# charlesyou999648/ARCO

Hardware: AMD Instinct MI355X
Metric: train steps/sec, ACDC 2D 256x256 bs=16 (higher is better)
Workload: dtype f32; 1 GPU; ACDC 2D 256x256 bs=16 per GPU on 1xMI355X, stratified sampler + 4096-key/class queue (BASELINE.json configs[1]), reference-default flags; classes=4, rep_dim=496, num_queries=256, num_negatives=512, func=smc, apply_aug=cutmix, loss_terms=k1*contrastive + k3*unsupervised + CE + Dice + k2*equivariance (k2 = 1), graph_train=1, parallelism=dp1

## Files before the change

arco_amd/csrc/conv_sp.hip:

```cpp
#include "igemm_args.h"
#include <stdlib.h>
#include <type_traits>

#include "sp_util.h"
__device__ __attribute__((aligned(64))) unsigned int conv_sp_zero_row[32];

template <int A_T, int C_T>
struct SpGeom {
  static constexpr int TH = 4 * A_T, HR = TH + 2, AROWS = HR * 18, BN = C_T * 16;
  static constexpr int A_DW = AROWS * 24;
  static constexpr int NBI = (2 * BN * 6 + 255) / 256;
  static constexpr int SLOT_DW = NBI * 256 * 4;
  static constexpr int NA_IT = (AROWS * 4 + 255) / 256;
  static constexpr int BIAS_DW = 256;
  static constexpr size_t LDS_BYTES = (size_t)(2 * A_DW + 5 * SLOT_DW + BIAS_DW) * 4;
};

template <int A_T, int C_T, bool PRO = false>
__global__ __launch_bounds__(512) void conv3x3_sp_kernel(IgemmArgs a) {
  using G = SpGeom<A_T, C_T>;
  constexpr int TH = G::TH, BN = G::BN, NA = G::NA_IT, NB = G::NBI;
  constexpr int NA4 = (NA + 3) / 4;
  constexpr int NL = NA + (PRO ? 4 : 0);
  extern __shared__ __attribute__((aligned(16))) float smem[];
  unsigned* const As = reinterpret_cast<unsigned*>(smem);
  unsigned* const Bs = As + 2 * G::A_DW;
  float* const bias_s = reinterpret_cast<float*>(Bs + 5 * G::SLOT_DW);

  const int tid = threadIdx.x & 255, lane = tid & 63, wid = tid >> 6, li = lane & 15, g = lane >> 4;
  const bool producer = threadIdx.x >= 256;
  const int tiles_x = a.W >> 4, tiles_y = a.H / TH, tiles_img = tiles_x * tiles_y;
  const int nchunks = a.K >> 4;
  const int total_tiles = a.n_mblocks * a.n_nblocks;
  const bool xcd_map = (gridDim.x & 7) == 0;
  const int G8 = xcd_map ? (int)gridDim.x >> 3 : (int)gridDim.x;
  const int T8 = xcd_map ? (total_tiles + 7) >> 3 : total_tiles;
  const int tile0 = xcd_map ? ((int)blockIdx.x & 7) * T8 + ((int)blockIdx.x >> 3) : (int)blockIdx.x;
  const int tile_end_x = xcd_map ? min(total_tiles, (((int)blockIdx.x & 7) + 1) * T8) : total_tiles;
  const int my_tiles = tile0 < tile_end_x ? (tile_end_x - tile0 + G8 - 1) / G8 : 0;
  const int total_gc = my_tiles * nchunks;
  if (my_tiles == 0) return;
  const bool has_stats = a.stat_sum != nullptr;

  struct Desc { int j, c, img, y0, x0, nblk, mblk, grp; };
  const int ipg = PRO ? a.NB / (a.pro.groups > 1 ? a.pro.groups : 1) : 1;
  auto decode = [&](Desc& d) {
    const int v = tile0 + d.j * G8;
    d.mblk = v / a.n_nblocks; d.nblk = v - d.mblk * a.n_nblocks;
    d.img = d.mblk / tiles_img;
    d.grp = PRO ? d.img / ipg : 0;
    const int r = d.mblk - d.img * tiles_img, ty = r / tiles_x;
    d.y0 = ty * TH; d.x0 = (r - ty * tiles_x) * 16;
  };
  auto advance = [&](Desc& d) { if (++d.c == nchunks) { d.c = 0; ++d.j; decode(d); } };
  Desc d0{0, 0, 0, 0, 0, 0, 0, 0};
  decode(d0);

  if (producer) {
    Desc d1 = d0; advance(d1);
    Desc d2 = d1; advance(d2);
    Desc d3 = d2; advance(d3);
    const int qA = tid & 3;
    int ldsA[NA]; unsigned voff[NA]; int poff[NA];
    unsigned m_valid = 0, m_top = 0, m_bot = 0, m_left = 0, m_right = 0;
#pragma unroll
    for (int it = 0; it < NA; ++it) {
      const int row = (tid + it * 256) >> 2;
      const int hy = row / 18, hx = row - hy * 18;
      const bool valid = row < G::AROWS;
      poff[it] = hy * a.W + hx;
      ldsA[it] = valid ? row * 24 + qA * 2 : -1;
      voff[it] = valid ? (unsigned)(((hy * a.W + hx) * (int)a.lda + qA * 4) * 4) : 0u;
      m_valid |= valid ? (1u << it) : 0u;
      m_top |= (valid && hy == 0) ? (1u << it) : 0u; m_bot |= (valid && hy == TH + 1) ? (1u << it) : 0u;
      m_left |= (valid && hx == 0) ? (1u << it) : 0u; m_right |= (valid && hx == 17) ? (1u << it) : 0u;
    }
    const unsigned safe_off = (unsigned)(((a.W + 1) * (int)a.lda + qA * 4) * 4);
    int woff[NB], wq[NB], wtap[NB];
#pragma unroll
    for (int i = 0; i < NB; ++i) {
      const int p = (i * 4 + wid) * 64 + lane;
      const int tl_ = p / (BN * 6), rem = p - tl_ * (BN * 6), n = rem / 6, q6 = rem - n * 6;
      wtap[i] = tl_ < 2 ? tl_ : 2;
      woff[i] = tl_ < 2 ? ((tl_ * a.Npad + n) * a.Kg) * 24 + q6 * 4 : 0;
      wq[i] = q6 * 4;
    }
    const long wslot2 = (long)2 * a.Npad * a.Kg * 24;
    const float* const zrow = reinterpret_cast<const float*>(conv_sp_zero_row);

    f32x4 ra[2][NA]; unsigned okm2[2] = {0, 0};
    f32x4 rp[2][4]; unsigned ebase2[2] = {0, 0}; bool bord2[2] = {true, true};
    const float* const pm_ = PRO ? uniform_ptr(a.pro.mean) : nullptr; const float* const pi_ = PRO ? uniform_ptr(a.pro.istd) : nullptr;
    const float* const pg_ = PRO ? uniform_ptr(a.pro.gamma) : nullptr; const float* const pb_ = PRO ? uniform_ptr(a.pro.beta) : nullptr;
    const bool pdrop = PRO && a.pro.drop_mode == 1;
    uint32_t dkey = 0, dthr = 0; float keep_scale = 1.f;
    u32x2 salt = {0u, 0u};
    if (PRO && pdrop && a.pro.seed_dev) {
      const float* sp_ = uniform_ptr(reinterpret_cast<const float*>(a.pro.seed_dev));
      asm volatile("global_load_dwordx2 %0, %1, %2" : "=v"(salt) : "v"(0u), "s"(sp_) : "memory");
    }
    auto drop_setup = [&]() {
      if (PRO && pdrop) {
        asm volatile("" : "+v"(salt)::"memory");
        const unsigned long long sv = ((unsigned long long)salt[1] << 32) | salt[0];
        const unsigned long long sd = a.pro.seed_dev ? a.pro.seed ^ (sv * 0x9E3779B97F4A7C15ull) : a.pro.seed;
        dkey = drop_key32(sd); dthr = drop_thr16(a.pro.p); keep_scale = 1.0f / (1.0f - a.pro.p);
      }
    };
    auto load_A = [&](const Desc& d, bool real, int set) {
      const float* gbase = uniform_ptr(real ? a.A + ((((long)d.img * a.H + d.y0 - 1) * a.W + d.x0 - 1) * a.lda + d.c * 16) : a.A);
      unsigned bad = (d.y0 == 0 ? m_top : 0u) | (d.y0 + TH == a.H ? m_bot : 0u) | (d.x0 == 0 ? m_left : 0u) | (d.x0 + 16 == a.W ? m_right : 0u);
      if (!real) bad = ~0u;
      const unsigned okm = m_valid & ~bad;
      okm2[set] = okm;
      const bool border = !real || d.y0 == 0 || d.y0 + TH == a.H || d.x0 == 0 || d.x0 + 16 == a.W;
      if constexpr (PRO) bord2[set] = border;
      if (!border) {
#pragma unroll
        for (int it = 0; it < NA; ++it) asm volatile("global_load_dwordx4 %0, %1, %2" : "=v"(ra[set][it]) : "v"(voff[it]), "s"(gbase) : "memory");
      } else {
#pragma unroll
        for (int it = 0; it < NA; ++it) {
          const unsigned o = ((okm >> it) & 1u) ? voff[it] : safe_off;
          asm volatile("global_load_dwordx4 %0, %1, %2" : "=v"(ra[set][it]) : "v"(o), "s"(gbase) : "memory");
        }
      }
      if constexpr (PRO) {
        const int ch = d.c * 16 + qA * 4;
        const unsigned po = (unsigned)(((real ? d.grp : 0) * a.K + ch) * 4), pa = (unsigned)(ch * 4);
        asm volatile("global_load_dwordx4 %0, %1, %2" : "=v"(rp[set][0]) : "v"(po), "s"(pm_) : "memory");
        asm volatile("global_load_dwordx4 %0, %1, %2" : "=v"(rp[set][1]) : "v"(po), "s"(pi_) : "memory");
        asm volatile("global_load_dwordx4 %0, %1, %2" : "=v"(rp[set][2]) : "v"(pa), "s"(pg_) : "memory");
        asm volatile("global_load_dwordx4 %0, %1, %2" : "=v"(rp[set][3]) : "v"(pa), "s"(pb_) : "memory");
        ebase2[set] = (unsigned)((((d.img * a.H + d.y0 - 1) * a.W + d.x0 - 1) * a.K) + ch);
      }
    };
    auto ra_fence = [&](int set) {
#pragma unroll
      for (int it = 0; it < NA; ++it) asm volatile("" : "+v"(ra[set][it])::"memory");
      if constexpr (PRO) {
#pragma unroll
        for (int j = 0; j < 4; ++j) asm volatile("" : "+v"(rp[set][j])::"memory");
      }
    };
    auto store_A = [&](unsigned* buf, int it, int set) {
      f32x4 v = ra[set][it];
      if constexpr (PRO) {
        v = pro_bn_lrelu(v, ProQuad{rp[set][0], rp[set][1], rp[set][2], rp[set][3]}, a.pro.slope);
        if (pdrop) v = pro_dropout(v, dkey, ebase2[set] + (unsigned)poff[it] * (unsigned)a.K, dthr, keep_scale);
        if (bord2[set]) v = pro_mask(v, okm2[set] >> it);
      } else {
        v = ((okm2[set] >> it) & 1u) ? v : f32x4{0, 0, 0, 0};
      }
      u32x2 p0, p1, p2;
      split3_bf16x4(v, p0, p1, p2);
      if (ldsA[it] >= 0) {
        unsigned* d = buf + ldsA[it];
        *reinterpret_cast<u32x2_ma*>(d) = p0; *reinterpret_cast<u32x2_ma*>(d + 8) = p1; *reinterpret_cast<u32x2_ma*>(d + 16) = p2;
      }
    };
    auto refill = [&](int slot, const Desc& d) {
      const float* base = a.Wp + slot * wslot2 + ((long)d.nblk * BN * a.Kg + d.c) * 24;
#pragma unroll
      for (int i = 0; i < NB; ++i) {
        const bool zero = wtap[i] == 2 || (slot == 4 && wtap[i] == 1);
        const float* src = zero ? zrow + wq[i] : base + woff[i];
        unsigned* dst = Bs + slot * G::SLOT_DW + (i * 4 + wid) * 256;
        __builtin_amdgcn_global_load_lds((glb_void_t*)src, (lds_void_t*)dst, 16, 0, 0);
      }
    };

    for (int i = tid; i < G::BIAS_DW; i += 256) bias_s[i] = (a.bias && i < a.N) ? a.bias[i] : 0.f;
    load_A(d0, true, 0);
    refill(0, d0); refill(1, d0); refill(2, d0);
    wait_vm<3 * NB>();
    drop_setup();
    ra_fence(0);
#pragma unroll
    for (int it = 0; it < NA; ++it) store_A(As, it, 0);
    refill(3, d0);
    load_A(d1, total_gc > 1, 1);
    load_A(d2, total_gc > 2, 0);
    wait_vm<NL>();
    wait_lgkm0();
    __builtin_amdgcn_s_barrier();

    auto pchunk = [&](auto SET_, int gc) {
      constexpr int SET = decltype(SET_)::value;
      const bool more = gc + 1 < total_gc;
      unsigned* Anxt = As + ((gc + 1) & 1) * G::A_DW;
      auto step = [&](auto S_) {
        constexpr int S = decltype(S_)::value;
        constexpr int NS = S <= 2 ? NL + 2 * NB : 2 * NB;
        wait_vm<NS>();
        wait_lgkm0();
        __builtin_amdgcn_s_barrier();
        refill(S == 0 ? 4 : S - 1, S == 0 ? d0 : (more ? d1 : d0));
        if (S == 0) ra_fence(SET);
        if (S <= 3) {
#pragma unroll
          for (int it = S * NA4; it < (S + 1) * NA4 && it < NA; ++it) store_A(Anxt, it, SET);
        }
        if (S == 4) load_A(d3, gc + 3 < total_gc, SET);
      };
      step(std::integral_constant<int, 0>{});
      step(std::integral_constant<int, 1>{});
      step(std::integral_constant<int, 2>{});
      step(std::integral_constant<int, 3>{});
      step(std::integral_constant<int, 4>{});
      d0 = d1; d1 = d2; d2 = d3; advance(d3);
    };
    for (int gc = 0; gc < total_gc; gc += 2) {
      pchunk(std::integral_constant<int, 1>{}, gc);
      if (gc + 1 < total_gc) pchunk(std::integral_constant<int, 0>{}, gc + 1);
    }
    wait_vm<0>();
    return;
  }

  const int tl = g >> 1;
  int aoff[5];
#pragma unroll
  for (int s = 0; s < 5; ++s) {
    const int tap = 2 * s + tl > 8 ? 8 : 2 * s + tl;
    aoff[s] = ((tap / 3) * 18 + tap % 3) * 24;
  }
  const int laneA = (wid * A_T * 18 + li) * 24 + (g & 1) * 4;
  const int laneB = (tl * BN + li) * 24 + (g & 1) * 4;
  bf16x8 fa[2][A_T][3], fb[2][3];
  f32x4 acc[A_T][C_T];
#pragma unroll
  for (int i = 0; i < A_T; ++i)
#pragma unroll
    for (int j = 0; j < C_T; ++j) acc[i][j] = f32x4{0, 0, 0, 0};

  __builtin_amdgcn_s_barrier();
#pragma unroll
  for (int at = 0; at < A_T; ++at)
#pragma unroll
    for (int pl = 0; pl < 3; ++pl) fa[0][at][pl] = lds_bf16x8(As + laneA + aoff[0] + at * 18 * 24 + 8 * pl);
#pragma unroll
  for (int pl = 0; pl < 3; ++pl) fb[0][pl] = lds_bf16x8(Bs + laneB + 8 * pl);

  auto chunk = [&](auto CP_, int gc) {
    constexpr int CP = decltype(CP_)::value;
    const unsigned* Acur = As + (gc & 1) * G::A_DW;
    const unsigned* Anxt = As + ((gc + 1) & 1) * G::A_DW;
    auto step = [&](auto S_) {
      constexpr int S = decltype(S_)::value;
      constexpr int P = (CP + S) & 1, Q = P ^ 1;
      wait_lgkm0();
      __builtin_amdgcn_s_barrier();
      constexpr int NCH = A_T * C_T;
      constexpr int APC = (A_T * 3 + (NCH - 2) - 1) / (NCH - 2 > 0 ? NCH - 2 : 1);
      const unsigned* An = S < 4 ? Acur : Anxt;
#pragma unroll
      for (int ct = 0; ct < C_T; ++ct) {
        constexpr int GB = (C_T & 1) ? (CP + S) : 0;
        const int BPc = (GB + ct) & 1, BPn = BPc ^ 1;
        const bool last = ct + 1 == C_T;
#pragma unroll
        for (int pl = 0; pl < 3; ++pl)
          fb[BPn][pl] = lds_bf16x8(Bs + (last ? (S + 1) % 5 : S) * G::SLOT_DW + laneB + (last ? 0 : ct + 1) * 16 * 24 + 8 * pl);
        __builtin_amdgcn_sched_barrier(0);
#pragma unroll
        for (int at = 0; at < A_T; ++at) {
          mfma_acc(acc[at][ct], fb[BPc][0], fa[P][at][2]);
          mfma_acc(acc[at][ct], fb[BPc][2], fa[P][at][0]);
          mfma_acc(acc[at][ct], fb[BPc][1], fa[P][at][1]);
          mfma_acc(acc[at][ct], fb[BPc][0], fa[P][at][1]);
          mfma_acc(acc[at][ct], fb[BPc][1], fa[P][at][0]);
          mfma_acc(acc[at][ct], fb[BPc][0], fa[P][at][0]);
          const int chain = ct * A_T + at;
#pragma unroll
          for (int k = chain * APC; k < (chain + 1) * APC && k < A_T * 3; ++k)
            fa[Q][k / 3][k % 3] = lds_bf16x8(An + laneA + aoff[(S + 1) % 5] + (k / 3) * 18 * 24 + 8 * (k % 3));
          __builtin_amdgcn_sched_barrier(0);
        }
      }
    };
    step(std::integral_constant<int, 0>{});
    step(std::integral_constant<int, 1>{});
    step(std::integral_constant<int, 2>{});
    step(std::integral_constant<int, 3>{});
    step(std::integral_constant<int, 4>{});
  };

  auto tile_end = [&]() {
    asm volatile("s_nop 15\n\ts_nop 15" ::: "memory");
    const int n0 = d0.nblk * BN;
    float s1[C_T][4], s2[C_T][4];
#pragma unroll
    for (int ct = 0; ct < C_T; ++ct) {
      const int n = n0 + ct * 16 + 4 * g;
      const f32x4 bv = *reinterpret_cast<const f32x4*>(bias_s + n);
#pragma unroll
      for (int r = 0; r < 4; ++r) { s1[ct][r] = 0.f; s2[ct][r] = 0.f; }
#pragma unroll
      for (int at = 0; at < A_T; ++at) {
        const long pix = ((long)d0.img * a.H + d0.y0 + wid * A_T + at) * a.W + d0.x0 + li;
        f32x4 v = acc[at][ct] + bv;
        if (a.R) v += *reinterpret_cast<const f32x4*>(a.R + pix * a.ldr + n);
        *reinterpret_cast<f32x4*>(a.C + pix * a.ldc + n) = v;
#pragma unroll
        for (int r = 0; r < 4; ++r) { s1[ct][r] += v[r]; s2[ct][r] += v[r] * v[r]; }
        acc[at][ct] = f32x4{0, 0, 0, 0};
      }
    }
    if (has_stats) {
      const long slab = (long)d0.mblk * 4 + wid, nslab = (long)a.n_mblocks * 4;
#pragma unroll
      for (int ct = 0; ct < C_T; ++ct)
#pragma unroll
        for (int r = 0; r < 4; ++r) {
          const float v1 = row16_sum(s1[ct][r]), v2 = row16_sum(s2[ct][r]);
          if (li == 0) {
            a.stat_sum[(n0 + ct * 16 + 4 * g + r) * nslab + slab] = v1;
            a.stat_sq[(n0 + ct * 16 + 4 * g + r) * nslab + slab] = v2;
          }
        }
    }
  };

  for (int gc = 0; gc < total_gc; gc += 2) {
    chunk(std::integral_constant<int, 0>{}, gc);
    if (d0.c + 1 == nchunks) tile_end();
    advance(d0);
    if (gc + 1 < total_gc) {
      chunk(std::integral_constant<int, 1>{}, gc + 1);
      if (d0.c + 1 == nchunks) tile_end();
      advance(d0);
    }
  }
}

template <int A_T, int C_T, int NCW = 4>
struct RwGeom {
  static constexpr int TH = NCW * A_T, AROWS = (TH + 2) * 18, BN = C_T * 16;
  static constexpr int A_DW = AROWS * 24;
  static constexpr int WCH_DW = 10 * BN * 24;
  static constexpr int NA_IT = (AROWS * 4 + 255) / 256;
  static constexpr int BIAS_DW = 64;
  static size_t lds_bytes(int nchunks) { return (size_t)(2 * A_DW + nchunks * WCH_DW + BIAS_DW) * 4; }
};

template <int A_T, int C_T, bool PRO = false, int NCW = 4>
__global__ __launch_bounds__((NCW + 4) * 64) void conv3x3_rw_kernel(IgemmArgs a) {
  using G = RwGeom<A_T, C_T, NCW>;
  constexpr int TH = G::TH, BN = G::BN, NA = G::NA_IT;
  constexpr int NL = NA + (PRO ? 4 : 0);
  extern __shared__ __attribute__((aligned(16))) float smem[];
  unsigned* const As = reinterpret_cast<unsigned*>(smem);
  const int nchunks = (a.K + 15) >> 4;
  unsigned* const Ws = As + 2 * G::A_DW;
  float* const bias_s = reinterpret_cast<float*>(Ws + nchunks * G::WCH_DW);
  const bool producer = threadIdx.x >= NCW * 64;
  const int tid = producer ? (int)threadIdx.x - NCW * 64 : (int)threadIdx.x, lane = tid & 63, wid = tid >> 6, li = lane & 15, g = lane >> 4;
  const int tiles_x = a.W >> 4, tiles_y = a.H / TH, tiles_img = tiles_x * tiles_y;
  const int total_tiles = a.n_mblocks;
  const bool xcd_map = (gridDim.x & 7) == 0;
  const int G8 = xcd_map ? (int)gridDim.x >> 3 : (int)gridDim.x;
  const int T8 = xcd_map ? (total_tiles + 7) >> 3 : total_tiles;
  const int tile0 = xcd_map ? ((int)blockIdx.x & 7) * T8 + ((int)blockIdx.x >> 3) : (int)blockIdx.x;
  const int tile_end_x = xcd_map ? min(total_tiles, (((int)blockIdx.x & 7) + 1) * T8) : total_tiles;
  const int my_tiles = tile0 < tile_end_x ? (tile_end_x - tile0 + G8 - 1) / G8 : 0;
  const int total_gc = my_tiles * nchunks;
  if (my_tiles == 0) return;
  const bool has_stats = a.stat_sum != nullptr;
  struct Desc { int j, c, img, y0, x0, mblk, grp; };
  const int ipg = PRO ? a.NB / (a.pro.groups > 1 ? a.pro.groups : 1) : 1;
  auto decode = [&](Desc& d) {
    d.mblk = tile0 + d.j * G8;
    d.img = d.mblk / tiles_img;
    d.grp = PRO ? d.img / ipg : 0;
    const int r = d.mblk - d.img * tiles_img, ty = r / tiles_x;
    d.y0 = ty * TH; d.x0 = (r - ty * tiles_x) * 16;
  };
  auto advance = [&](Desc& d) { if (++d.c == nchunks) { d.c = 0; ++d.j; decode(d); } };
  Desc d0{0, 0, 0, 0, 0, 0, 0};
  decode(d0);

  if (producer) {
    const float* const zrow = reinterpret_cast<const float*>(conv_sp_zero_row);
    const int wpieces = nchunks * 10 * BN * 6;
    for (int p0 = wid * 64; p0 < wpieces; p0 += 256) {
      const int p = p0 + lane;
      const int q6 = p % 6, row = p / 6, n = row % BN, tp = (row / BN) % 10, c = row / (BN * 10);
      const float* src = (tp < 9 && p < wpieces) ? a.Wp + (((long)tp * a.Npad + n) * a.Kg + c) * 24 + q6 * 4 : zrow + q6 * 4;
      __builtin_amdgcn_global_load_lds((glb_void_t*)src, (lds_void_t*)(Ws + p0 * 4), 16, 0, 0);
    }
    for (int i = tid; i < G::BIAS_DW; i += 256) bias_s[i] = (a.bias && i < a.N) ? a.bias[i] : 0.f;
    Desc d1 = d0; advance(d1);
    Desc d2 = d1; advance(d2);
    Desc d3 = d2; advance(d3);
    const int qA = tid & 3;
    int ldsA[NA]; unsigned voff[NA]; int poff[NA];
    unsigned m_valid = 0, m_top = 0, m_bot = 0, m_left = 0, m_right = 0;
#pragma unroll
    for (int it = 0; it < NA; ++it) {
      const int row = (tid + it * 256) >> 2;
      const int hy = row / 18, hx = row - hy * 18;
      const bool valid = row < G::AROWS;
      poff[it] = hy * a.W + hx;
      ldsA[it] = valid ? row * 24 + qA * 2 : -1;
      voff[it] = valid ? (unsigned)(((hy * a.W + hx) * (int)a.lda + qA * 4) * 4) : 0u;
      m_valid |= valid ? (1u << it) : 0u;
      m_top |= (valid && hy == 0) ? (1u << it) : 0u; m_bot |= (valid && hy == TH + 1) ? (1u << it) : 0u;
      m_left |= (valid && hx == 0) ? (1u << it) : 0u; m_right |= (valid && hx == 17) ? (1u << it) : 0u;
    }
    const unsigned safe_off = (unsigned)(((a.W + 1) * (int)a.lda + qA * 4) * 4);
    f32x4 ra[2][NA]; unsigned okm2[2] = {0, 0};
    f32x4 rp[2][4]; unsigned ebase2[2] = {0, 0}; bool bord2[2] = {true, true};
    const float* const pm_ = PRO ? uniform_ptr(a.pro.mean) : nullptr; const float* const pi_ = PRO ? uniform_ptr(a.pro.istd) : nullptr;
    const float* const pg_ = PRO ? uniform_ptr(a.pro.gamma) : nullptr; const float* const pb_ = PRO ? uniform_ptr(a.pro.beta) : nullptr;
    const bool pdrop = PRO && a.pro.drop_mode == 1;
    uint32_t dkey = 0, dthr = 0; float keep_scale = 1.f;
    u32x2 salt = {0u, 0u};
    if (PRO && pdrop && a.pro.seed_dev) {
      const float* sp_ = uniform_ptr(reinterpret_cast<const float*>(a.pro.seed_dev));
      asm volatile("global_load_dwordx2 %0, %1, %2" : "=v"(salt) : "v"(0u), "s"(sp_) : "memory");
    }
    auto drop_setup = [&]() {
      if (PRO && pdrop) {
        asm volatile("" : "+v"(salt)::"memory");
        const unsigned long long sv = ((unsigned long long)salt[1] << 32) | salt[0];
        const unsigned long long sd = a.pro.seed_dev ? a.pro.seed ^ (sv * 0x9E3779B97F4A7C15ull) : a.pro.seed;
        dkey = drop_key32(sd); dthr = drop_thr16(a.pro.p); keep_scale = 1.0f / (1.0f - a.pro.p);
      }
    };
    auto load_A = [&](const Desc& d, bool real, int set) {
      const float* gbase = uniform_ptr(real ? a.A + ((((long)d.img * a.H + d.y0 - 1) * a.W + d.x0 - 1) * a.lda + d.c * 16) : a.A);
      unsigned bad = (d.y0 == 0 ? m_top : 0u) | (d.y0 + TH == a.H ? m_bot : 0u) | (d.x0 == 0 ? m_left : 0u) | (d.x0 + 16 == a.W ? m_right : 0u);
      if (!real || d.c * 16 + qA * 4 >= a.K) bad = ~0u;
      okm2[set] = m_valid & ~bad;
      const bool border = !real || d.y0 == 0 || d.y0 + TH == a.H || d.x0 == 0 || d.x0 + 16 == a.W || d.c * 16 + 16 > a.K;
      if constexpr (PRO) bord2[set] = border;
#ifdef RW_NO_LOAD
      if (true) { (void)gbase; } else
#endif
      if (!border) {
#pragma unroll
        for (int it = 0; it < NA; ++it) asm volatile("global_load_dwordx4 %0, %1, %2" : "=v"(ra[set][it]) : "v"(voff[it]), "s"(gbase) : "memory");
      } else {
        const unsigned okm = okm2[set];
#pragma unroll
        for (int it = 0; it < NA; ++it) {
          const unsigned o = ((okm >> it) & 1u) ? voff[it] : safe_off;
          asm volatile("global_load_dwordx4 %0, %1, %2" : "=v"(ra[set][it]) : "v"(o), "s"(gbase) : "memory");
        }
      }
      if constexpr (PRO) {
        const int ch = d.c * 16 + qA * 4;
        const unsigned po = (unsigned)(((real ? d.grp : 0) * a.K + (ch < a.K ? ch : 0)) * 4), pa = (unsigned)((ch < a.K ? ch : 0) * 4);
        asm volatile("global_load_dwordx4 %0, %1, %2" : "=v"(rp[set][0]) : "v"(po), "s"(pm_) : "memory");
        asm volatile("global_load_dwordx4 %0, %1, %2" : "=v"(rp[set][1]) : "v"(po), "s"(pi_) : "memory");
        asm volatile("global_load_dwordx4 %0, %1, %2" : "=v"(rp[set][2]) : "v"(pa), "s"(pg_) : "memory");
        asm volatile("global_load_dwordx4 %0, %1, %2" : "=v"(rp[set][3]) : "v"(pa), "s"(pb_) : "memory");
        ebase2[set] = (unsigned)((((d.img * a.H + d.y0 - 1) * a.W + d.x0 - 1) * a.K) + ch);
      }
    };
    auto store_all = [&](unsigned* buf, int set) {
#pragma unroll
      for (int it = 0; it < NA; ++it) asm volatile("" : "+v"(ra[set][it])::"memory");
      ProQuad pq;
      if constexpr (PRO) {
#pragma unroll
        for (int j = 0; j < 4; ++j) asm volatile("" : "+v"(rp[set][j])::"memory");
        pq = ProQuad{rp[set][0], rp[set][1], rp[set][2], rp[set][3]};
      }
      const unsigned okm = okm2[set];
#pragma unroll
      for (int it = 0; it < NA; ++it) {
        f32x4 v = ra[set][it];
        if constexpr (PRO) {
          v = pro_bn_lrelu(v, pq, a.pro.slope);
          if (pdrop) v = pro_dropout(v, dkey, ebase2[set] + (unsigned)poff[it] * (unsigned)a.K, dthr, keep_scale);
          if (bord2[set]) v = pro_mask(v, okm >> it);
        } else {
          v = ((okm >> it) & 1u) ? v : f32x4{0, 0, 0, 0};
        }
        u32x2 p0, p1, p2;
#ifdef RW_NO_SPLIT
        p0 = u32x2{__float_as_uint(v[0]), __float_as_uint(v[1])}; p1 = u32x2{__float_as_uint(v[2]), __float_as_uint(v[3])}; p2 = p0;
#else
        split3_bf16x4(v, p0, p1, p2);
#endif
        if (ldsA[it] >= 0) {
          unsigned* d = buf + ldsA[it];
          *reinterpret_cast<u32x2_ma*>(d) = p0; *reinterpret_cast<u32x2_ma*>(d + 8) = p1; *reinterpret_cast<u32x2_ma*>(d + 16) = p2;
        }
      }
    };
    load_A(d0, true, 0);
    load_A(d1, total_gc > 1, 1);
    wait_vm<NL>();
    drop_setup();
    store_all(As, 0);
    load_A(d2, total_gc > 2, 0);
    wait_lgkm0();
    __builtin_amdgcn_s_barrier();
    wait_vm<NL>();
    store_all(As + G::A_DW, 1);
    load_A(d3, total_gc > 3, 1);
    Desc dn = d3; advance(dn);
    for (int k = 0; k < total_gc; k += 2) {
      wait_lgkm0();
      __builtin_amdgcn_s_barrier();
      wait_vm<NL>();
      store_all(As, 0);
      load_A(dn, k + 4 < total_gc, 0);
      advance(dn);
      if (k + 1 < total_gc) {
        wait_lgkm0();
        __builtin_amdgcn_s_barrier();
        wait_vm<NL>();
        store_all(As + G::A_DW, 1);
        load_A(dn, k + 5 < total_gc, 1);
        advance(dn);
      }
    }
    wait_vm<0>();
    return;
  }

  const int tl = g >> 1;
  int aoff[5];
#pragma unroll
  for (int s_ = 0; s_ < 5; ++s_) {
    const int tap = 2 * s_ + tl > 8 ? 8 : 2 * s_ + tl;
    aoff[s_] = ((tap / 3) * 18 + tap % 3) * 24;
  }
  const int laneA = (wid * A_T * 18 + li) * 24 + (g & 1) * 4;
  const int laneB = (tl * BN + li) * 24 + (g & 1) * 4;
  bf16x8 fa[A_T][3], fb[2][C_T][3];
  f32x4 acc[A_T][C_T];
#pragma unroll
  for (int i = 0; i < A_T; ++i)
#pragma unroll
    for (int j = 0; j < C_T; ++j) acc[i][j] = f32x4{0, 0, 0, 0};
  __builtin_amdgcn_s_barrier();
#pragma unroll
  for (int at = 0; at < A_T; ++at)
#pragma unroll
    for (int pl = 0; pl < 3; ++pl) fa[at][pl] = lds_bf16x8(As + laneA + aoff[0] + at * 18 * 24 + 8 * pl);
#pragma unroll
  for (int ct = 0; ct < C_T; ++ct)
#pragma unroll
    for (int pl = 0; pl < 3; ++pl) fb[0][ct][pl] = lds_bf16x8(Ws + laneB + ct * 16 * 24 + 8 * pl);

  auto chunk = [&](auto CP_, int gc, int c, bool more) {
    constexpr int CP = decltype(CP_)::value;
    const unsigned* Acur = As + (gc & 1) * G::A_DW;
    const unsigned* Anxt = As + ((gc + 1) & 1) * G::A_DW;
    const unsigned* Wc = Ws + c * G::WCH_DW;
    const unsigned* Wn = Ws + (c + 1 == nchunks ? 0 : c + 1) * G::WCH_DW;
    auto step = [&](auto S_) {
      constexpr int S = decltype(S_)::value;
      constexpr int P = (CP + S) & 1, Q = P ^ 1;
      if (S == 4) {
        wait_lgkm0();
        __builtin_amdgcn_s_barrier();
      }
      constexpr int BPA = (C_T * 3 + A_T - 1) / A_T;
      const unsigned* An = S < 4 ? Acur : Anxt;
      const unsigned* Wb = (S < 4 ? Wc : Wn) + ((S + 1) % 5) * (2 * BN * 24);
#pragma unroll
      for (int at = 0; at < A_T; ++at) {
#pragma unroll
        for (int ct = 0; ct < C_T; ++ct) {
#ifdef RW_NO_MFMA
          asm volatile("" :: "v"(fb[P][ct][0]), "v"(fb[P][ct][1]), "v"(fb[P][ct][2]), "v"(fa[at][0]), "v"(fa[at][1]), "v"(fa[at][2]));
          continue;
#endif
          mfma_acc(acc[at][ct], fb[P][ct][0], fa[at][2]);
          mfma_acc(acc[at][ct], fb[P][ct][2], fa[at][0]);
          mfma_acc(acc[at][ct], fb[P][ct][1], fa[at][1]);
          mfma_acc(acc[at][ct], fb[P][ct][0], fa[at][1]);
          mfma_acc(acc[at][ct], fb[P][ct][1], fa[at][0]);
          mfma_acc(acc[at][ct], fb[P][ct][0], fa[at][0]);
        }
#ifndef RW_NO_FRAG
        if (S < 4 || more) {
#pragma unroll
          for (int pl = 0; pl < 3; ++pl) fa[at][pl] = lds_bf16x8(An + laneA + aoff[(S + 1) % 5] + at * 18 * 24 + 8 * pl);
        }
#pragma unroll
        for (int k = at * BPA; k < (at + 1) * BPA && k < C_T * 3; ++k)
          fb[Q][k / 3][k % 3] = lds_bf16x8(Wb + laneB + (k / 3) * 16 * 24 + 8 * (k % 3));
#else
        (void)An; (void)Wb;
#endif
        __builtin_amdgcn_sched_barrier(0);
      }
    };
    step(std::integral_constant<int, 0>{});
    step(std::integral_constant<int, 1>{});
    step(std::integral_constant<int, 2>{});
    step(std::integral_constant<int, 3>{});
    step(std::integral_constant<int, 4>{});
  };
  auto tile_end = [&]() {
    asm volatile("s_nop 15\n\ts_nop 15" ::: "memory");
    float s1[C_T][4], s2[C_T][4];
#pragma unroll
    for (int ct = 0; ct < C_T; ++ct) {
      const int n = ct * 16 + 4 * g;
      const f32x4 bv = *reinterpret_cast<const f32x4*>(bias_s + n);
#pragma unroll
      for (int r = 0; r < 4; ++r) { s1[ct][r] = 0.f; s2[ct][r] = 0.f; }
#pragma unroll
      for (int at = 0; at < A_T; ++at) {
        const long pix = ((long)d0.img * a.H + d0.y0 + wid * A_T + at) * a.W + d0.x0 + li;
        f32x4 v = acc[at][ct] + bv;
        if (n < a.N) {
          if (a.R) v += *reinterpret_cast<const f32x4*>(a.R + pix * a.ldr + n);
#ifdef RW_NO_STORE
          if (v[0] == 1.2345e30f)
#endif
          *reinterpret_cast<f32x4*>(a.C + pix * a.ldc + n) = v;
        }
#pragma unroll
        for (int r = 0; r < 4; ++r) { s1[ct][r] += v[r]; s2[ct][r] += v[r] * v[r]; }
        acc[at][ct] = f32x4{0, 0, 0, 0};
      }
    }
    if (has_stats) {
      const long slab = (long)d0.mblk * NCW + wid, nslab = (long)a.n_mblocks * NCW;
#pragma unroll
      for (int ct = 0; ct < C_T; ++ct)
#pragma unroll
        for (int r = 0; r < 4; ++r) {
          const float v1 = row16_sum(s1[ct][r]), v2 = row16_sum(s2[ct][r]);
          if (li == 0 && ct * 16 + 4 * g < a.N) {
            a.stat_sum[(ct * 16 + 4 * g + r) * nslab + slab] = v1;
            a.stat_sq[(ct * 16 + 4 * g + r) * nslab + slab] = v2;
          }
        }
    }
  };
  for (int gc = 0; gc < total_gc; gc += 2) {
    chunk(std::integral_constant<int, 0>{}, gc, d0.c, gc + 1 < total_gc);
    if (d0.c + 1 == nchunks) tile_end();
    advance(d0);
    if (gc + 1 < total_gc) {
      chunk(std::integral_constant<int, 1>{}, gc + 1, d0.c, gc + 2 < total_gc);
      if (d0.c + 1 == nchunks) tile_end();
      advance(d0);
    }
  }
}

template <int A_T, int C_T, int NCW>
static int launch_rw(const IgemmArgs& a, hipStream_t st, int* q) {
  using G = RwGeom<A_T, C_T, NCW>;
  const int mblocks = a.NB * (a.H / G::TH) * (a.W / 16);
  if (q) { q[0] = NCW * mblocks; q[1] = 9350000 + (G::TH / 4) * 1000 + G::BN; q[2] = 1610; return ARCO_OK; }
  if ((a.ldc & 3) != 0 || (a.R && (a.ldr & 3) != 0)) return ARCO_ERR_UNSUPPORTED;
  arco_note_route(9350000 + (G::TH / 4) * 1000 + G::BN);
  const size_t lds = G::lds_bytes((a.K + 15) >> 4);
  IgemmArgs b = a;
  b.n_mblocks = mblocks; b.n_nblocks = 1;
  const int cus = conv_sp_cus();
  if (a.pro.mean) {
    if ((a.K & 15) != 0) return ARCO_ERR_UNSUPPORTED;
    auto kern = conv3x3_rw_kernel<A_T, C_T, true, NCW>;
    static unsigned long long attr_set = 0;
    if (arco_first_on_device(attr_set)) { (void)hipFuncSetAttribute(reinterpret_cast<const void*>(kern), hipFuncAttributeMaxDynamicSharedMemorySize, 160 * 1024); }
    hipLaunchKernelGGL(kern, dim3((unsigned)(mblocks < cus ? mblocks : cus)), dim3((NCW + 4) * 64), lds, st, b);
    return arco_launch_status();
  }
  auto kern = conv3x3_rw_kernel<A_T, C_T, false, NCW>;
  static unsigned long long attr_set = 0;
  if (arco_first_on_device(attr_set)) { (void)hipFuncSetAttribute(reinterpret_cast<const void*>(kern), hipFuncAttributeMaxDynamicSharedMemorySize, 160 * 1024); }
  hipLaunchKernelGGL(kern, dim3((unsigned)(mblocks < cus ? mblocks : cus)), dim3((NCW + 4) * 64), lds, st, b);
  return arco_launch_status();
}

template <int A_T, int C_T>
static int launch_sp(const IgemmArgs& a, hipStream_t st, int* q) {
  using G = SpGeom<A_T, C_T>;
  const int mblocks = a.NB * (a.H / G::TH) * (a.W / 16);
  if (q) { q[0] = 4 * mblocks; q[1] = 9300000 + A_T * 1000 + G::BN; q[2] = 1610; return ARCO_OK; }
  if ((a.ldc & 3) != 0 || (a.R && (a.ldr & 3) != 0)) return ARCO_ERR_UNSUPPORTED;
  arco_note_route(9300000 + A_T * 1000 + G::BN);
  IgemmArgs b = a;
  b.n_mblocks = mblocks; b.n_nblocks = a.Npad / G::BN;
  const int total = mblocks * b.n_nblocks, cus = conv_sp_cus();
  if (a.pro.mean) {
    auto kern = conv3x3_sp_kernel<A_T, C_T, true>;
    static unsigned long long attr_set = 0;
    if (arco_first_on_device(attr_set)) { (void)hipFuncSetAttribute(reinterpret_cast<const void*>(kern), hipFuncAttributeMaxDynamicSharedMemorySize, (int)G::LDS_BYTES); }
    hipLaunchKernelGGL(kern, dim3((unsigned)(total < cus ? total : cus)), dim3(512), G::LDS_BYTES, st, b);
    return arco_launch_status();
  }
  auto kern = conv3x3_sp_kernel<A_T, C_T>;
  static unsigned long long attr_set = 0;
  if (arco_first_on_device(attr_set)) { (void)hipFuncSetAttribute(reinterpret_cast<const void*>(kern), hipFuncAttributeMaxDynamicSharedMemorySize, (int)G::LDS_BYTES); }
  hipLaunchKernelGGL(kern, dim3((unsigned)(total < cus ? total : cus)), dim3(512), G::LDS_BYTES, st, b);
  return arco_launch_status();
}


struct Rw3Geom {
  static constexpr int TH = 16, HR = (TH + 2) * 18, NT = 512, NW = 8;
  static constexpr int WROWS = 27 * 16 + 1;
  static constexpr int W_DW = WROWS * 24, A_DW = HR * 24;
  static constexpr int NP = (HR * 4 + NT - 1) / NT;
  static constexpr size_t LDS_BYTES = (size_t)(W_DW + 3 * A_DW + 2 * NW * 16) * 4;
};

__global__ __launch_bounds__(512) void conv3d_rw16_kernel(IgemmArgs a, int S, int nseg) {
  using G = Rw3Geom;
  constexpr int HR = G::HR, WROWS = G::WROWS, NP = G::NP, NT = G::NT, NW = G::NW, TH = G::TH;
  extern __shared__ __attribute__((aligned(16))) float smem[];
  unsigned* const Ws = reinterpret_cast<unsigned*>(smem);
  unsigned* const As = Ws + G::W_DW;
  float* const red = reinterpret_cast<float*>(As + 3 * G::A_DW);
  const int tid = threadIdx.x, lane = tid & 63, wid = tid >> 6, li = lane & 15, g = lane >> 4, h = g >> 1;
  const int tiles_x = a.W >> 4, tiles_y = a.H / TH;
  const int units = (a.NB / a.D3) * tiles_y * tiles_x * nseg;

  for (int i = tid; i < (WROWS - 1) * 6; i += NT) {
    const int r = i / 6, q6 = i - r * 6;
    *reinterpret_cast<u32x4_ma*>(Ws + r * 24 + q6 * 4) = *reinterpret_cast<const u32x4*>(a.Wp + ((long)r * a.Kg) * 24 + q6 * 4);
  }
  for (int i = tid; i < 24; i += NT) Ws[(WROWS - 1) * 24 + i] = 0u;

  int prow[NP], pq[NP];
#pragma unroll
  for (int i = 0; i < NP; ++i) {
    const int idx = tid + i * NT;
    prow[i] = idx < HR * 4 ? idx >> 2 : -1; pq[i] = idx & 3;
  }
  f32x4 bv;
#pragma unroll
  for (int r = 0; r < 4; ++r) bv[r] = a.bias ? a.bias[4 * g + r] : 0.f;

  f32x4 R[NP];
  const bool xmap = (gridDim.x & 7) == 0;
  const int G8 = xmap ? (int)gridDim.x >> 3 : (int)gridDim.x, U8 = xmap ? (units + 7) >> 3 : units;
  const int u_lo = xmap ? ((int)blockIdx.x & 7) * U8 : 0, u_hi = xmap ? min(units, u_lo + U8) : units;
  for (int unit = u_lo + (xmap ? (int)blockIdx.x >> 3 : (int)blockIdx.x); unit < u_hi; unit += G8) {
    const int seg = unit % nseg; int col = unit / nseg;
    const int tx = col % tiles_x; col /= tiles_x;
    const int ty = col % tiles_y; const int v = col / tiles_y;
    const int y0 = ty * TH, x0 = tx * 16, p0 = seg * S, p1 = min(a.D3, p0 + S);
    auto load_plane = [&](int p) {
      const bool pok = p >= 0 && p < a.D3;
#pragma unroll
      for (int i = 0; i < NP; ++i) {
        f32x4 val = f32x4{0, 0, 0, 0};
        if (prow[i] >= 0 && pok) {
          const int hy = prow[i] / 18, hx = prow[i] - hy * 18;
          const int y = y0 + hy - 1, x = x0 + hx - 1;
          if (y >= 0 && y < a.H && x >= 0 && x < a.W)
            val = *reinterpret_cast<const f32x4*>(a.A + ((((long)v * a.D3 + p) * a.H + y) * a.W + x) * a.lda + pq[i] * 4);
        }
        R[i] = val;
      }
    };
    auto store_plane = [&](int slot) {
#pragma unroll
      for (int i = 0; i < NP; ++i)
        if (prow[i] >= 0) {
          u32x2 p0_, p1_, p2_;
          split3_bf16x4(R[i], p0_, p1_, p2_);
          unsigned* d = As + slot * G::A_DW + prow[i] * 24 + pq[i] * 2;
          *reinterpret_cast<u32x2_ma*>(d) = p0_; *reinterpret_cast<u32x2_ma*>(d + 8) = p1_; *reinterpret_cast<u32x2_ma*>(d + 16) = p2_;
        }
    };
    f32x4 t1 = {0, 0, 0, 0}, t2 = {0, 0, 0, 0};
    int sA = 0, sB = 1, sC = 2;
    load_plane(p0 - 1); store_plane(sA);
    load_plane(p0); store_plane(sB);
    load_plane(p0 + 1);
    for (int p = p0; p < p1; ++p) {
      store_plane(sC);
      __syncthreads();
      if (p + 1 < p1) load_plane(p + 2);
      f32x4 acc[2] = {f32x4{0, 0, 0, 0}, f32x4{0, 0, 0, 0}};
      const int sb0 = sA * G::A_DW, sb1 = sB * G::A_DW, sb2 = sC * G::A_DW;
      bf16x8 fb[2][3], fa[2][2][3];
      auto read_step = [&](int sp_, int set) {
        const int tp0 = 2 * sp_, tp1 = 2 * sp_ + 1 > 26 ? 26 : 2 * sp_ + 1;
        const int dz0 = tp0 / 9, dz1 = tp1 / 9;
        const int o0 = ((tp0 % 9) / 3) * 18 + tp0 % 3, o1 = ((tp1 % 9) / 3) * 18 + tp1 % 3;
        const int base0 = (dz0 == 0 ? sb0 : (dz0 == 1 ? sb1 : sb2)) + o0 * 24;
        const int base1 = (dz1 == 0 ? sb0 : (dz1 == 1 ? sb1 : sb2)) + o1 * 24;
        const int abase = (h ? base1 : base0) + (g & 1) * 4;
        const int wrow = h ? (2 * sp_ + 1 > 26 ? WROWS - 1 : tp1 * 16 + li) : tp0 * 16 + li;
#pragma unroll
        for (int pl = 0; pl < 3; ++pl) fb[set][pl] = lds_bf16x8(Ws + wrow * 24 + (g & 1) * 4 + 8 * pl);
#pragma unroll
        for (int at = 0; at < 2; ++at)
#pragma unroll
          for (int pl = 0; pl < 3; ++pl) fa[set][at][pl] = lds_bf16x8(As + abase + ((2 * wid + at) * 18 + li) * 24 + 8 * pl);
      };
      read_step(0, 0);
#pragma unroll
      for (int s = 0; s < 14; ++s) {
        if (s + 1 < 14) read_step(s + 1, (s + 1) & 1);
        __builtin_amdgcn_sched_barrier(0);
#pragma unroll
        for (int at = 0; at < 2; ++at) {
          f32x4 c = acc[at];
          c = __builtin_amdgcn_mfma_f32_16x16x32_bf16(fb[s & 1][0], fa[s & 1][at][2], c, 0, 0, 0);
          c = __builtin_amdgcn_mfma_f32_16x16x32_bf16(fb[s & 1][2], fa[s & 1][at][0], c, 0, 0, 0);
          c = __builtin_amdgcn_mfma_f32_16x16x32_bf16(fb[s & 1][1], fa[s & 1][at][1], c, 0, 0, 0);
          c = __builtin_amdgcn_mfma_f32_16x16x32_bf16(fb[s & 1][0], fa[s & 1][at][1], c, 0, 0, 0);
          c = __builtin_amdgcn_mfma_f32_16x16x32_bf16(fb[s & 1][1], fa[s & 1][at][0], c, 0, 0, 0);
          c = __builtin_amdgcn_mfma_f32_16x16x32_bf16(fb[s & 1][0], fa[s & 1][at][0], c, 0, 0, 0);
          acc[at] = c;
        }
        __builtin_amdgcn_sched_barrier(0);
      }
#pragma unroll
      for (int at = 0; at < 2; ++at) {
        const long pix = ((((long)v * a.D3 + p) * a.H + y0 + 2 * wid + at) * a.W + x0 + li);
        const f32x4 o = acc[at] + bv;
        *reinterpret_cast<f32x4*>(a.C + pix * a.ldc + 4 * g) = o;
        t1 += o; t2 += o * o;
      }
      __syncthreads();
      const int t = sA; sA = sB; sB = sC; sC = t;
    }
    if (a.stat_sum) {
#pragma unroll
      for (int r = 0; r < 4; ++r) {
        const float v1 = row16_sum(t1[r]), v2 = row16_sum(t2[r]);
        if (li == 0) { red[(0 * NW + wid) * 16 + 4 * g + r] = v1; red[(1 * NW + wid) * 16 + 4 * g + r] = v2; }
      }
      __syncthreads();
      if (tid < 16) {
        float v1 = 0.f, v2 = 0.f;
#pragma unroll
        for (int w = 0; w < NW; ++w) { v1 += red[(0 * NW + w) * 16 + tid]; v2 += red[(1 * NW + w) * 16 + tid]; }
        for (int p = p0; p < p1; ++p) {
          const long slab = (((long)v * a.D3 + p) * tiles_y + ty) * tiles_x + tx;
          a.stat_sum[(long)tid * a.n_mblocks + slab] = p == p0 ? v1 : 0.f;
          a.stat_sq[(long)tid * a.n_mblocks + slab] = p == p0 ? v2 : 0.f;
        }
      }
      __syncthreads();
    }
  }
}

int conv3d_rw_dispatch(const IgemmArgs& a, hipStream_t st, int* q) {
  if (a.mma != 3 || a.K != 16 || a.N != 16 || a.Npad != 16 || a.Kg != 2 || (a.H & 15) != 0 || (a.W & 15) != 0 ||
      (a.lda & 3) != 0 || (a.ldc & 3) != 0 || a.R != nullptr) return -1;
  using G = Rw3Geom;
  const long tiles = (long)(a.H / G::TH) * (a.W >> 4);
  if (q) { q[0] = (int)(a.NB * tiles); q[1] = 9 * 1000000 + 450000 + 16; q[2] = 16 * 100 + 30 + 1; return ARCO_OK; }
  if (a.D3 < 1 || a.NB % a.D3 != 0) return ARCO_ERR_ARG;
  const long cols = (long)(a.NB / a.D3) * tiles, slots = conv_sp_cus();
  int S = 8;
  while (S > 2 && cols * ((a.D3 + S - 1) / S) < 3 * slots) S >>= 1;
  if (S > a.D3) S = a.D3;
  const int nseg = (a.D3 + S - 1) / S;
  const long units = cols * nseg;
  static unsigned long long attr_set = 0;
  if (arco_first_on_device(attr_set)) { (void)hipFuncSetAttribute(reinterpret_cast<const void*>(conv3d_rw16_kernel), hipFuncAttributeMaxDynamicSharedMemorySize, (int)G::LDS_BYTES); }
  IgemmArgs b = a;
  b.n_mblocks = (int)(a.NB * tiles);
  arco_note_route(9 * 1000000 + 450000 + 16);
  hipLaunchKernelGGL(conv3d_rw16_kernel, dim3((unsigned)(slots < units ? slots : units)), dim3(G::NT), G::LDS_BYTES, st, b, S, nseg);
  return arco_launch_status();
}

static int& conv_sp_flag() { static int on = 1; return on; }
static bool conv_sp_on() { return conv_sp_flag() != 0; }
extern "C" int arco_conv_sp_set(int on) { const int prev = conv_sp_flag(); conv_sp_flag() = on ? 1 : 0; return prev; }

template <int C_T>
static int dispatch_rows(const IgemmArgs& a, hipStream_t st, int* q, int min_tiles) {
  const long cols = (long)a.NB * (a.W / 16) * (a.N / (16 * C_T));
  if (cols * (a.H / 16) >= min_tiles) return launch_sp<4, C_T>(a, st, q);
  if ((a.H & 7) == 0 && cols * (a.H / 8) >= min_tiles) return launch_sp<2, C_T>(a, st, q);
  if ((a.H & 3) == 0 && cols * (a.H / 4) >= min_tiles) return launch_sp<1, C_T>(a, st, q);
  return -1;
}

constexpr int CONV_SP_MIN_TILES = 192;
int conv_sp_dispatch(const IgemmArgs& a, hipStream_t st, int* q) {
  if (!conv_sp_on() || a.mma != 3 || a.D3 != 1) return -1;
  if ((a.lda & 3) != 0 || (a.W & 15) != 0 || (a.H & 3) != 0) return -1;
  constexpr int min_tiles = CONV_SP_MIN_TILES;
  if (a.Npad == 16 && (a.N & 3) == 0 && a.K <= 32 && (a.K & 3) == 0 && ((a.K & 15) == 0 || a.K < 16) &&
      (a.H & 31) == 0 && (long)a.NB * (a.H / 32) * (a.W / 16) >= min_tiles) {
    return launch_rw<4, 1, 8>(a, st, q);
  }
  if ((a.K & 15) != 0 || a.K < 16 || (a.N & 15) != 0 || a.N != a.Npad || a.N > 256) return -1;
  if (a.K <= 32 && a.N == 32 && (a.H & 15) == 0 && (long)a.NB * (a.H / 16) * (a.W / 16) >= min_tiles)
    return launch_rw<2, 2, 8>(a, st, q);
  if ((a.N & 63) == 0) return dispatch_rows<4>(a, st, q, min_tiles);
  if ((a.N & 31) == 0) return dispatch_rows<2>(a, st, q, min_tiles);
  return (a.H & 15) == 0 ? launch_sp<4, 1>(a, st, q) : -1;
}
```

Before: 93.85 steps/s (16-image steps, all GPUs).

## Accumulate BN statistics per workgroup across tiles instead of per-tile slabs

The persistent 3x3 conv kernel now keeps running per-channel sum and sum-of-squares in registers across all tiles a workgroup processes. It writes one slab per workgroup per stat group instead of one per tile per wave, and zero-fills the slots of groups it never touches. This shrinks the stat buffer and the later reduction work in the batch-norm stats kernel. The cost is extra registers, more bookkeeping, and a dependence on the reducer and the slab-count query (q[0]) agreeing with the new layout.

```diff
diff --git a/arco_amd/csrc/conv_sp.hip b/arco_amd/csrc/conv_sp.hip
--- a/arco_amd/csrc/conv_sp.hip
+++ b/arco_amd/csrc/conv_sp.hip
@@ -4,6 +4,14 @@
 
 #include "sp_util.h"
 __device__ __attribute__((aligned(64))) unsigned int conv_sp_zero_row[32];
+
+__device__ __forceinline__ void stat_zero_groups(const IgemmArgs& a, int waves, int g0, int g1, int wid) {
+  const long wg_slabs = (long)gridDim.x * waves, nslab = (a.stat_groups > 1 ? a.stat_groups : 1) * wg_slabs;
+  for (int sg = g0; sg < g1; ++sg) {
+    const long slot = sg * wg_slabs + (long)blockIdx.x * waves + wid;
+    for (int c = (int)__lane_id(); c < a.N; c += 64) { a.stat_sum[c * nslab + slot] = 0.f; a.stat_sq[c * nslab + slot] = 0.f; }
+  }
+}
 
 template <int A_T, int C_T>
 struct SpGeom {
@@ -365,8 +373,13 @@
   const int tile_end_x = xcd_map ? min(total_tiles, (((int)blockIdx.x & 7) + 1) * T8) : total_tiles;
   const int my_tiles = tile0 < tile_end_x ? (tile_end_x - tile0 + G8 - 1) / G8 : 0;
   const int total_gc = my_tiles * nchunks;
-  if (my_tiles == 0) return;
   const bool has_stats = a.stat_sum != nullptr;
+  if (my_tiles == 0) {
+#ifndef ARCO_STAT_PER_TILE
+    if (has_stats && !producer) stat_zero_groups(a, NCW, 0, a.stat_groups > 1 ? a.stat_groups : 1, wid);
+#endif
+    return;
+  }
   struct Desc { int j, c, img, y0, x0, mblk, grp; };
   const int ipg = PRO ? a.NB / (a.pro.groups > 1 ? a.pro.groups : 1) : 1;
   auto decode = [&](Desc& d) {
@@ -538,6 +551,19 @@
   for (int i = 0; i < A_T; ++i)
 #pragma unroll
     for (int j = 0; j < C_T; ++j) acc[i][j] = f32x4{0, 0, 0, 0};
+#ifndef ARCO_STAT_PER_TILE
+  float S1[C_T][4], S2[C_T][4];
+#pragma unroll
+  for (int ct = 0; ct < C_T; ++ct)
+#pragma unroll
+    for (int r = 0; r < 4; ++r) { S1[ct][r] = 0.f; S2[ct][r] = 0.f; }
+  int gend;
+  {
+    const int n_sg = a.stat_groups > 1 ? a.stat_groups : 1, mpg = total_tiles / n_sg, sgrp = d0.mblk / mpg;
+    gend = (sgrp + 1) * mpg;
+    if (has_stats) stat_zero_groups(a, NCW, 0, sgrp, wid);
+  }
+#endif
   __builtin_amdgcn_s_barrier();
 #pragma unroll
   for (int at = 0; at < A_T; ++at)
@@ -599,7 +625,7 @@
     step(std::integral_constant<int, 3>{});
     step(std::integral_constant<int, 4>{});
   };
-  auto tile_end = [&]() {
+  auto tile_end = [&](bool last) {
     asm volatile("s_nop 15\n\ts_nop 15" ::: "memory");
     float s1[C_T][4], s2[C_T][4];
 #pragma unroll
@@ -623,7 +649,12 @@
         for (int r = 0; r < 4; ++r) { s1[ct][r] += v[r]; s2[ct][r] += v[r] * v[r]; }
         acc[at][ct] = f32x4{0, 0, 0, 0};
       }
-    }
+#ifndef ARCO_STAT_PER_TILE
+#pragma unroll
+      for (int r = 0; r < 4; ++r) { S1[ct][r] += s1[ct][r]; S2[ct][r] += s2[ct][r]; }
+#endif
+    }
+#ifdef ARCO_STAT_PER_TILE
     if (has_stats) {
       const long slab = (long)d0.mblk * NCW + wid, nslab = (long)a.n_mblocks * NCW;
 #pragma unroll
@@ -637,42 +668,77 @@
           }
         }
     }
+#else
+    if (last || d0.mblk + G8 >= gend) {
+      if (has_stats) {
+        int n_sg = a.stat_groups > 1 ? a.stat_groups : 1;
+        asm volatile("" : "+s"(n_sg));
+        const int mpg = total_tiles / n_sg, sgrp = gend / mpg - 1, wg_slabs = (int)gridDim.x * NCW;
+        const long slot = (long)sgrp * wg_slabs + (int)blockIdx.x * NCW + wid, ns = (long)n_sg * wg_slabs;
+#pragma unroll
+        for (int ct = 0; ct < C_T; ++ct)
+#pragma unroll
+          for (int r = 0; r < 4; ++r) {
+            const float v1 = row16_sum(S1[ct][r]), v2 = row16_sum(S2[ct][r]);
+            S1[ct][r] = 0.f; S2[ct][r] = 0.f;
+            if (li == 0 && ct * 16 + 4 * g < a.N) {
+              a.stat_sum[(ct * 16 + 4 * g + r) * ns + slot] = v1;
+              a.stat_sq[(ct * 16 + 4 * g + r) * ns + slot] = v2;
+            }
+          }
+        const int g_n = last ? n_sg : (d0.mblk + G8) / mpg;
+        stat_zero_groups(a, NCW, sgrp + 1, g_n, wid);
+        gend = (g_n + 1) * mpg;
+      }
+    }
+#endif
   };
   for (int gc = 0; gc < total_gc; gc += 2) {
     chunk(std::integral_constant<int, 0>{}, gc, d0.c, gc + 1 < total_gc);
-    if (d0.c + 1 == nchunks) tile_end();
+    if (d0.c + 1 == nchunks) tile_end(gc + 1 == total_gc);
     advance(d0);
     if (gc + 1 < total_gc) {
       chunk(std::integral_constant<int, 1>{}, gc + 1, d0.c, gc + 2 < total_gc);
-      if (d0.c + 1 == nchunks) tile_end();
+      if (d0.c + 1 == nchunks) tile_end(gc + 2 == total_gc);
       advance(d0);
     }
   }
+}
+
+static int stat_slabs(const IgemmArgs& a, int mblocks, int grid, int waves) {
+#ifdef ARCO_STAT_PER_TILE
+  return waves * mblocks;
+#else
+  return (a.stat_groups > 1 ? a.stat_groups : 1) * grid * waves;
+#endif
 }
 
 template <int A_T, int C_T, int NCW>
 static int launch_rw(const IgemmArgs& a, hipStream_t st, int* q) {
   using G = RwGeom<A_T, C_T, NCW>;
   const int mblocks = a.NB * (a.H / G::TH) * (a.W / 16);
-  if (q) { q[0] = NCW * mblocks; q[1] = 9350000 + (G::TH / 4) * 1000 + G::BN; q[2] = 1610; return ARCO_OK; }
+  const int cus = conv_sp_cus(), grid = mblocks < cus ? mblocks : cus;
+  if (q) {
+    q[0] = stat_slabs(a, mblocks, grid, NCW); q[1] = 9350000 + (G::TH / 4) * 1000 + G::BN; q[2] = 1610;
+    return ARCO_OK;
+  }
   if ((a.ldc & 3) != 0 || (a.R && (a.ldr & 3) != 0)) return ARCO_ERR_UNSUPPORTED;
   arco_note_route(9350000 + (G::TH / 4) * 1000 + G::BN);
   const size_t lds = G::lds_bytes((a.K + 15) >> 4);
   IgemmArgs b = a;
   b.n_mblocks = mblocks; b.n_nblocks = 1;
-  const int cus = conv_sp_cus();
   if (a.pro.mean) {
     if ((a.K & 15) != 0) return ARCO_ERR_UNSUPPORTED;
     auto kern = conv3x3_rw_kernel<A_T, C_T, true, NCW>;
     static unsigned long long attr_set = 0;
     if (arco_first_on_device(attr_set)) { (void)hipFuncSetAttribute(reinterpret_cast<const void*>(kern), hipFuncAttributeMaxDynamicSharedMemorySize, 160 * 1024); }
-    hipLaunchKernelGGL(kern, dim3((unsigned)(mblocks < cus ? mblocks : cus)), dim3((NCW + 4) * 64), lds, st, b);
+    hipLaunchKernelGGL(kern, dim3((unsigned)grid), dim3((NCW + 4) * 64), lds, st, b);
     return arco_launch_status();
   }
   auto kern = conv3x3_rw_kernel<A_T, C_T, false, NCW>;
   static unsigned long long attr_set = 0;
   if (arco_first_on_device(attr_set)) { (void)hipFuncSetAttribute(reinterpret_cast<const void*>(kern), hipFuncAttributeMaxDynamicSharedMemorySize, 160 * 1024); }
-  hipLaunchKernelGGL(kern, dim3((unsigned)(mblocks < cus ? mblocks : cus)), dim3((NCW + 4) * 64), lds, st, b);
+  hipLaunchKernelGGL(kern, dim3((unsigned)grid), dim3((NCW + 4) * 64), lds, st, b);
   return arco_launch_status();
 }
 
```

Result: no change. 94.07 steps/s (16-image steps, all GPUs), median of 2 (+0.2%).
